# JiangongChen/ORB_SLAM3-1

Hardware: AMD Instinct MI355X
Metric: tracking frames/s (ORB extract+match) (higher is better)
Workload: dtype u8; 1 GPU; ORBextractor 640x480, 8 levels, 1000 features (configs[1]) + SearchByBoW 1000x1000 per frame (configs[2]); batch_per_gpu=256

## Files before the change

### include/orbslam3_hip.h

```cpp
#ifndef ORBSLAM3_HIP_H
#define ORBSLAM3_HIP_H

#include <stddef.h>
#include <stdint.h>

#ifdef __cplusplus
extern "C" {
#endif

#define ORBX_OK 0
#define ORBX_ERR_EMPTY (-1)
#define ORBX_ERR_CAPACITY (-2)
#define ORBX_ERR_ARG (-3)
#define ORBX_ERR_NO_DEVICE (-4)
#define ORBX_ERR_HIP (-5)
#define ORBX_ERR_INTERNAL (-6)

const char* orbx_last_error(void);
int orbx_device_count(void);


typedef struct OrbxKeyPoint {
    float x, y;
    float size;
// ... 19 lines not shown
                              int row_stride, size_t frame_stride, int lap0, int lap1,
                              OrbxKeyPoint* d_kps, uint8_t* d_desc, int cap, int32_t* d_n, int32_t* d_mono,
                              int32_t* d_status, void* stream);

int orbx_max_keypoints(const orbx_extractor* h);
int orbx_max_keypoints_for(const orbx_extractor* h, int width, int height);

int orbx_levels(const orbx_extractor* h);
float orbx_scale_factor(const orbx_extractor* h);
int orbx_scale_tables(const orbx_extractor* h, float* scale, float* inv_scale, float* sigma2, float* inv_sigma2);
int orbx_features_per_level(const orbx_extractor* h, int* n_per_level);

int orbx_pyramid_level_size(const orbx_extractor* h, int level, int* width, int* height);
int orbx_pyramid_level(orbx_extractor* h, int frame, int level, int border, uint8_t* dst, int dst_stride);

int orbx_stereo_matches(orbx_extractor* left, orbx_extractor* right, int frame,
                        const OrbxKeyPoint* kps_l, const uint8_t* desc_l, int n_l,
                        const OrbxKeyPoint* kps_r, const uint8_t* desc_r, int n_r, float mb, float mbf, float* u_right, float* depth);
int orbx_stereo_matches_device(orbx_extractor* left, orbx_extractor* right, int batch,
                               const OrbxKeyPoint* d_kps_l, const uint8_t* d_desc_l, const int32_t* d_n_l,
                               const OrbxKeyPoint* d_kps_r, const uint8_t* d_desc_r, const int32_t* d_n_r, int cap,
                               float mb, float mbf, float* d_u_right, float* d_depth, void* stream);

int orbx_profile_enable(orbx_extractor* h, int on);
int orbx_profile_read(orbx_extractor* h, float* stage_ms, int n_stages);

int orbx_debug_blurred_level(orbx_extractor* h, int frame, int level, uint8_t* dst, int dst_stride);
int orbx_debug_candidates(orbx_extractor* h, int frame, int level, OrbxKeyPoint* out, int cap, int* n);
int orbx_debug_level_keypoints(orbx_extractor* h, int frame, int level, OrbxKeyPoint* out, int cap, int* n);
int orbx_debug_set_fast_corner_cap(orbx_extractor* h, int cap);
int orbx_debug_set_tail_delay(orbx_extractor* h, int microseconds);
int orbx_debug_last_schedule(orbx_extractor* h);
int orbx_debug_fast_scores(const uint8_t* patches, int n, int pitch, int* out);


int orbm_hamming(const uint8_t a[32], const uint8_t b[32]);

typedef struct OrbmFeatVec {
    int32_t n_nodes;
    const uint32_t* node_id;
    const int32_t* offset;
    const uint32_t* feat;
} OrbmFeatVec;

typedef struct orbm_matcher orbm_matcher;
int orbm_create(int device, orbm_matcher** out);
void orbm_destroy(orbm_matcher* m);

int orbm_search_by_bow(orbm_matcher* m,
                       const uint8_t* desc_kf, int n_kf, const uint8_t* valid_kf, const float* angle_kf, const OrbmFeatVec* fv_kf,
                       const uint8_t* desc_f, int n_f, const float* angle_f, const OrbmFeatVec* fv_f,
                       float nnratio, int check_orientation, int32_t* match_f2kf);

typedef struct OrbmBowPair {
    const uint8_t* desc_kf; int32_t n_kf; const uint8_t* valid_kf; const float* angle_kf; OrbmFeatVec fv_kf;
    const uint8_t* desc_f;  int32_t n_f;  const float* angle_f;  OrbmFeatVec fv_f;
    int32_t* match_f2kf;
    int32_t n_matches;
} OrbmBowPair;
int orbm_search_by_bow_batch(orbm_matcher* m, OrbmBowPair* pairs, int n_pairs, float nnratio, int check_orientation);

typedef struct orbm_bow_plan orbm_bow_plan;
int orbm_bow_plan_create(orbm_matcher* m, const OrbmBowPair* pairs, int n_pairs, orbm_bow_plan** out);
int orbm_bow_plan_run(orbm_bow_plan* plan, float nnratio, int check_orientation, void* stream);
int orbm_bow_plan_fetch(orbm_bow_plan* plan, OrbmBowPair* pairs, void* stream);
void orbm_bow_plan_destroy(orbm_bow_plan* plan);
// ... 485 lines not shown
```

### orb_slam3-1_amd/capi.py

```python
import ctypes as C
import os

import numpy as np

_PKG_DIR = os.path.dirname(os.path.abspath(__file__))
_LIB_PATH = os.path.join(_PKG_DIR, "liborbslam3_hip.so")

KP_DTYPE = np.dtype([("x", "f4"), ("y", "f4"), ("size", "f4"), ("angle", "f4"), ("response", "f4"),
                     ("octave", "i4"), ("class_id", "i4")])
assert KP_DTYPE.itemsize == 28

ORBX_OK, ORBX_ERR_EMPTY, ORBX_ERR_CAPACITY, ORBX_ERR_ARG, ORBX_ERR_NO_DEVICE, ORBX_ERR_HIP, ORBX_ERR_INTERNAL = 0, -1, -2, -3, -4, -5, -6


class OrbxError(RuntimeError):
    def __init__(self, code, msg):
        super().__init__("orbslam3_hip error %d: %s" % (code, msg))
        self.code = code


class FeatVec(C.Structure):
    _fields_ = [("n_nodes", C.c_int32), ("node_id", C.c_void_p), ("offset", C.c_void_p), ("feat", C.c_void_p)]


# ... 29 lines not shown
    if not os.path.exists(_LIB_PATH):
        raise ImportError("%s not found: build it with __graft_entry__.build() (hipcc, gfx950). "
                          "There is no CPU fallback." % _LIB_PATH)
    return C.CDLL(_LIB_PATH)


lib = _load()
lib.orbx_last_error.restype = C.c_char_p
lib.orbx_create.argtypes = [C.c_int, C.c_float, C.c_int, C.c_int, C.c_int, C.c_int, C.POINTER(C.c_void_p)]
lib.orbx_destroy.argtypes = [C.c_void_p]
lib.orbx_extract.argtypes = [C.c_void_p, C.c_void_p, C.c_int, C.c_int, C.c_int, C.c_int, C.c_int,
                             C.c_void_p, C.c_void_p, C.c_int, C.POINTER(C.c_int), C.POINTER(C.c_int)]
lib.orbx_extract_batch.argtypes = [C.c_void_p, C.POINTER(C.c_void_p), C.c_int, C.c_int, C.c_int, C.c_int, C.c_int, C.c_int,
                                   C.c_void_p, C.c_void_p, C.c_int, C.c_void_p, C.c_void_p]
lib.orbx_extract_batch_device.argtypes = [C.c_void_p, C.c_void_p, C.c_int, C.c_int, C.c_int, C.c_int, C.c_size_t, C.c_int, C.c_int,
                                          C.c_void_p, C.c_void_p, C.c_int, C.c_void_p, C.c_void_p, C.c_void_p, C.c_void_p]
lib.orbx_max_keypoints.argtypes = [C.c_void_p]
lib.orbx_max_keypoints_for.argtypes = [C.c_void_p, C.c_int, C.c_int]
lib.orbx_levels.argtypes = [C.c_void_p]
lib.orbx_scale_factor.argtypes = [C.c_void_p]
lib.orbx_scale_factor.restype = C.c_float
lib.orbx_scale_tables.argtypes = [C.c_void_p] + [C.c_void_p] * 4
lib.orbx_features_per_level.argtypes = [C.c_void_p, C.c_void_p]
lib.orbx_pyramid_level_size.argtypes = [C.c_void_p, C.c_int, C.POINTER(C.c_int), C.POINTER(C.c_int)]
lib.orbx_pyramid_level.argtypes = [C.c_void_p, C.c_int, C.c_int, C.c_int, C.c_void_p, C.c_int]
lib.orbx_debug_blurred_level.argtypes = [C.c_void_p, C.c_int, C.c_int, C.c_void_p, C.c_int]
lib.orbx_debug_candidates.argtypes = [C.c_void_p, C.c_int, C.c_int, C.c_void_p, C.c_int, C.POINTER(C.c_int)]
lib.orbx_debug_level_keypoints.argtypes = [C.c_void_p, C.c_int, C.c_int, C.c_void_p, C.c_int, C.POINTER(C.c_int)]
lib.orbx_debug_set_tail_delay.argtypes = [C.c_void_p, C.c_int]
lib.orbx_debug_last_schedule.argtypes = [C.c_void_p]
lib.orbx_debug_introsort.argtypes = [C.c_void_p, C.c_void_p, C.c_void_p, C.c_int]
lib.orbx_debug_wave_sort.argtypes = [C.c_void_p, C.c_void_p, C.c_void_p, C.c_int]
lib.orbx_debug_fast_scores.argtypes = [C.c_void_p, C.c_int, C.c_int, C.c_void_p]
lib.orbx_debug_fast_atan2.restype = C.c_float
lib.orbx_debug_fast_atan2.argtypes = [C.c_float, C.c_float]
lib.orbx_debug_sincos.argtypes = [C.c_float, C.POINTER(C.c_float), C.POINTER(C.c_float)]


def _p(a):
    return None if a is None else a.ctypes.data_as(C.c_void_p)


def _check(code):
    if code < 0:
        raise OrbxError(code, (lib.orbx_last_error() or b"").decode())
    return code


def device_count():
    return lib.orbx_device_count()


class Extractor:

    def __init__(self, nfeatures=1000, scale_factor=1.2, nlevels=8, ini_th_fast=20, min_th_fast=7, device=0):
        h = C.c_void_p()
        _check(lib.orbx_create(nfeatures, scale_factor, nlevels, ini_th_fast, min_th_fast, device, C.byref(h)))
        self._h = h
        self.nlevels = nlevels
        self.max_keypoints = lib.orbx_max_keypoints(h)

    def close(self):
        if getattr(self, "_h", None):
            lib.orbx_destroy(self._h)
            self._h = None

# ... 1895 lines not shown
```

### orb_slam3-1_amd/csrc/orbx_device.h

```cpp
#pragma once

#include <stddef.h>
#include <stdint.h>

#include "../../include/orbslam3_hip.h"

namespace orbx {

constexpr int kEdge = 19;
constexpr int kHalfPatch = 15;
constexpr int kPatch = 31;
constexpr int kMaxLevels = 16;
constexpr int kOctLogFactor = 6;

struct LevelDesc {
    int32_t w, h, stride;
    int32_t nfeat;
    int64_t off;
    int32_t cell_begin, cell_count;
    int32_t cand_off, cand_cap;
    int32_t sel_off, sel_cap;
    float scale;
    int32_t patch_size;
};

struct CellDesc {
    int16_t level;
    int16_t x0, y0, x1, y1;
    int32_t slot_off, slot_cap;
};

struct TileDesc {
    int16_t level, x0, y0;
    int16_t edge;
};

struct __attribute__((aligned(16))) ResizeRow {
    uint32_t sy, b0, b1, pad;
};

__host__ __device__ inline int xcd_grid(int n_items) { return 8 * ((n_items + 7) / 8); }
__host__ __device__ inline int xcd_remap(int block, int grid, int frame)
{
    const int chunk = grid >> 3;
    return (((block & 7) + frame) & 7) * chunk + (block >> 3);
}

__host__ __device__ inline uint32_t pack_key(uint32_t x, uint32_t y, uint32_t resp) { return (x << 20) | (y << 8) | resp; }
__host__ __device__ inline uint32_t key_x(uint32_t e) { return e >> 20; }
__host__ __device__ inline uint32_t key_y(uint32_t e) { return (e >> 8) & 0xFFFu; }
__host__ __device__ inline uint32_t key_resp(uint32_t e) { return e & 0xFFu; }

}
```

### orb_slam3-1_amd/csrc/orbx_extractor.hip

```cpp
#include <hip/hip_runtime.h>

#include <algorithm>
#include <cmath>
#include <cstdarg>
#include <cstdio>
#include <cstdlib>
#include <cstring>
#include <string>
#include <vector>

#include "hip_check.h"
#include "orbx_kernels.hip"

namespace orbx {

thread_local std::string g_last_error;

int fail(int code, const char* fmt, ...)
{
    char buf[512];
    va_list ap;
    va_start(ap, fmt);
    vsnprintf(buf, sizeof(buf), fmt, ap);
    va_end(ap);
// ... 32 lines not shown
    {
        if (count <= n) return ORBX_OK;
        if (p) { (void)hipFree(p); p = nullptr; n = 0; }
        ORBX_HIP(hipMalloc((void**)&p, count * sizeof(T)));
        n = count;
        return ORBX_OK;
    }
    int upload(const std::vector<T>& v)
    {
        int r = ensure(v.size() ? v.size() : 1);
        if (r) return r;
        if (!v.empty()) ORBX_HIP(hipMemcpy(p, v.data(), v.size() * sizeof(T), hipMemcpyHostToDevice));
        return ORBX_OK;
    }
    void release() { if (p) (void)hipFree(p); p = nullptr; n = 0; }
};

}

using namespace orbx;

struct orbx_extractor {
    int device = 0;
    int nfeatures = 0, nlevels = 0, ini_th = 0, min_th = 0;
    float scale_factor_f = 0;
    double scale_factor_d = 0;
    std::vector<float> scale, inv_scale, sigma2, inv_sigma2;
    std::vector<int> nfeat;
    int taps[7];
    int max_kp = 0;

    int geo_w = 0, geo_h = 0;
    std::vector<LevelDesc> levels;
    std::vector<CellDesc> cells;
    std::vector<TileDesc> tiles;
    size_t pyr_frame_bytes = 0;
    int cand_frame_entries = 0, sel_frame_entries = 0;
    std::vector<StripDesc> strips;
    std::vector<StripRec> strip_recs;
    FastLds fast_layout;
    int fast_corner_cap = 0;
    size_t fast_lds = 0, oct_lds = 0;
    int oct_pool = 0, oct_lds_keys = 0, oct_small_keys = 0;
    bool oct_nodes_hbm = false;
    size_t oct_node_stride = 0;
    size_t oct_small_lds = 0;
    int oct_dyn_keys = 0;
    size_t oct_dyn_lds = 0;
    bool oct_keys_forced = false;

    DevBuf<LevelDesc> d_levels;
    DevBuf<CellDesc> d_cells;
    DevBuf<TileDesc> d_tiles;
    DevBuf<StripRec> d_strips;
    std::vector<DevBuf<int> > d_qsx0;
    std::vector<DevBuf<uint4> > d_qsel, d_qalpha;
    std::vector<DevBuf<ResizeRow> > d_rows;
    std::vector<DevBuf<int> > d_xofs, d_yofs;
    std::vector<DevBuf<short> > d_ialpha, d_ibeta;
    std::vector<uint8_t> resize_generic;

    int batch_cap = 0, last_batch = 0;
    DevBuf<uint8_t> d_pyr, d_blur;
    DevBuf<uint32_t> d_cand, d_scratch, d_sel;
    DevBuf<uint8_t> d_oct_nodes;
    DevBuf<int> d_cell_count, d_sel_count, d_kp_dst;
// ... 186 lines not shown
                qsx0[q] = xofs[4 * q];
                uint32_t se[4], al[4];
                for (int k = 0; k < 4; k++) {
                    const int dx = 4 * q + k;
                    if (dx < L.w) {
                        const int o = xofs[dx] - qsx0[q];
                        if (o < 0) return fail(ORBX_ERR_INTERNAL, "resize table: source offset %d", o);
                        if (o > 6) { resize_generic[l] = 1; se[k] = 0x0C0C0C0Cu; al[k] = 0u; continue; }
                        se[k] = (uint32_t)o | 0x0C000C00u | ((uint32_t)(o + 1) << 16);
                        al[k] = (uint32_t)(uint16_t)ia[2 * dx] | ((uint32_t)(uint16_t)ia[2 * dx + 1] << 16);
                    } else { se[k] = 0x0C0C0C0Cu; al[k] = 0u; }
                }
                qsel[q] = make_uint4(se[0], se[1], se[2], se[3]);
                qal[q] = make_uint4(al[0], al[1], al[2], al[3]);
            }
            std::vector<ResizeRow> rows((size_t)round_up(L.h, kResizeRows));
            for (size_t dy = 0; dy < rows.size(); dy++) {
                const int y = std::min((int)dy, L.h - 1);
                const int sy0 = std::min(std::max(yofs[y], 0), P.h - 1), sy1 = std::min(std::max(yofs[y] + 1, 0), P.h - 1);
                if (ib[2 * y] < 0 || ib[2 * y] > 2048 || ib[2 * y + 1] < 0 || ib[2 * y + 1] > 2048)
                    return fail(ORBX_ERR_INTERNAL, "resize table: row coefficients %d %d", ib[2 * y], ib[2 * y + 1]);
                rows[dy].sy = (uint32_t)sy0 | ((uint32_t)sy1 << 16);
                rows[dy].b0 = (uint32_t)ib[2 * y] << 12; rows[dy].b1 = (uint32_t)ib[2 * y + 1] << 12; rows[dy].pad = 0;
            }
            int r;
            if (resize_generic[l] && ((r = d_xofs[l].upload(xofs)) || (r = d_ialpha[l].upload(ia)) || (r = d_yofs[l].upload(yofs)) || (r = d_ibeta[l].upload(ib)))) return r;
            if ((r = d_qsx0[l].upload(qsx0)) || (r = d_qsel[l].upload(qsel)) || (r = d_qalpha[l].upload(qal)) || (r = d_rows[l].upload(rows))) return r;
        }
    }
    pyr_frame_bytes = off;
    if (off >= ((size_t)1 << 31)) return fail(ORBX_ERR_ARG, "the pyramid of a %dx%d image exceeds 2 GiB per frame", w, h);
    cand_frame_entries = std::max(cand_off, 1);
    sel_frame_entries = sel_off;
    {
        if (cells.size() > 32767) return fail(ORBX_ERR_ARG, "%zu FAST cells exceed the strip table's 16-bit cell index", cells.size());
        int max_nch = 1, max_ngx = 1, max_sth = 7, max_ent = 1, max_ncell = 1, max_int = 1;
        for (const StripDesc& sd : strips) {
            const int g0 = (sd.x0 + 3) >> 2, g1 = (sd.x1 - 4) >> 2, ngx = g1 - g0 + 1, sth = sd.y1 - sd.y0, ih = sth - 6;
            if (ngx > 64 || ih > 127) return fail(ORBX_ERR_ARG, "FAST strip of %dx%d px exceeds the 64-quad x 127-row work item index", sd.x1 - sd.x0, sth);
            const int xa = (4 * (g0 - 1)) & ~15, qoff = 4 * g0 - xa;
            max_nch = std::max(max_nch, (qoff + 4 * ngx + 4 + 15) >> 4);
            for (int j = 0; j < sd.ncell; j++) { const CellDesc& c = cells[sd.cell0 + j]; max_int = std::max(max_int, (c.x1 - c.x0 - 6) * ih); }
            max_ngx = std::max(max_ngx, ngx); max_sth = std::max(max_sth, sth);
            max_ent = std::max(max_ent, ((ih + 3) / 4) * (ngx + sd.ncell - 1));
            max_ncell = std::max(max_ncell, (int)sd.ncell);
        }
        if (max_int > 8191) return fail(ORBX_ERR_ARG, "FAST cell interior of %d px exceeds the 8191-px bitmask", max_int);
        FastLds& Z = fast_layout;
        auto al16 = [](size_t v) { return (v + 15) & ~(size_t)15; };
        size_t o = 0;
        Z.tile_pitch = 16 * max_nch;
        o = al16((size_t)max_sth * Z.tile_pitch);
        Z.map_off = (int)o; Z.map_pitch = 4 * max_ngx + 8;
        o = al16(o + (size_t)(max_sth - 6 + 2) * Z.map_pitch);
        Z.ent_cap = (max_ent + 7) & ~7;
        Z.ent_off = (int)o; o = al16(o + 2 * 4 * (size_t)Z.ent_cap);
        Z.px_off = (int)o; o = al16(o + 2 * 4 * (size_t)kPxCap);
        Z.corner_cap = fast_corner_cap > 0 ? fast_corner_cap : kCornerCap;
        Z.corner_off = (int)o; o = al16(o + 2 * 4 * (size_t)Z.corner_cap);
        Z.wpc = (max_int + 31) / 32;
        Z.pre_off = (int)o; o = al16(o + 4 * (size_t)max_ncell * Z.wpc);
        Z.bits_off = (int)o; o = al16(o + 4 * (size_t)max_ncell * Z.wpc);
        Z.total = (int)o;
        fast_lds = o;
        if (fast_lds > 150 * 1024) return fail(ORBX_ERR_ARG, "FAST strip of %d quads x %d rows does not fit LDS", max_ngx, max_sth);
        strip_recs.assign(strips.size(), StripRec());
// ... 237 lines not shown
            if (n_cells > 0) launch_fast(s, 0, (int)strips.size());
        }
        ORBX_LAUNCHED("k_fast_strips");
        if (marks) mark();
        hipStream_t os = blur_s ? blur_s : s;
        if (blur_s) {
            ORBX_HIP(hipEventRecord(ev_fork, s));
            ORBX_HIP(hipStreamWaitEvent(blur_s, ev_fork, 0));
        }
        if (two_launches) {
            ORBX_HIP(hipStreamWaitEvent(oct_stream, ev_fork, 0));
            {
                const int k_hi = dyn_keys ? std::max(64, o_keys / 2) : 0;
                launch_octree(oct_stream, oct_split, nlevels, oct_lds_hi + 8 * (size_t)k_hi, oct_pool_hi, k_hi);
            }
            ORBX_HIP(hipEventRecord(ev_oct_join, oct_stream));
        }
        launch_octree(os, oct0_early ? 1 : 0, lv_lo, o_lds, oct_pool, o_keys);
        if (blur_s) {
            if (tail_beside) ORBX_HIP(hipStreamWaitEvent(s, ev_tail, 0));
            launch_blur(s);
        }
        last_octree_variant = (oct_nodes_hbm ? 0 : (dyn_keys ? 3 : (o_keys > 0 ? 1 : 2))) | (two_launches ? 4 : 0) | (oct0_early ? 8 : 0) | (in_place ? 16 : 0) | (tail_beside ? 32 : 0) | (chain_beside ? 64 : 0);
        if (two_launches) ORBX_HIP(hipStreamWaitEvent(os, ev_oct_join, 0));
        ORBX_LAUNCHED("k_octree / k_blur");
        if (marks) mark();
        hipLaunchKernelGGL(k_index, dim3(nB), dim3(64), 0, os, d_levels.p, nlevels, sel, sel_frame_entries, sel_cnt,
                           lap0, lap1, cap, kp_dst, sel_frame_entries, o_n + f0, o_mono + f0, o_status + f0);
        ORBX_LAUNCHED("k_index");
        if (marks) mark();
        if (blur_s) { ORBX_HIP(hipEventRecord(ev_join, blur_s)); ORBX_HIP(hipStreamWaitEvent(s, ev_join, 0)); }
        else launch_blur(s);
        if (marks) mark();
        hipLaunchKernelGGL(k_orient_desc, dim3((unsigned)(((long long)quads * nB + 7) / 8 * 8)), dim3(256), 0, s, pyr, blr, pyr_frame_bytes,
                           d_levels.p, nlevels, sel, sel_frame_entries, sel_cnt, kp_dst, sel_frame_entries,
                           o_kps + (size_t)f0 * cap, o_desc + (size_t)f0 * cap * 32, cap, d_lvl_kps.p + (size_t)f0 * sel_frame_entries, quads, nB);
        ORBX_LAUNCHED("k_orient_desc");
        if (marks) mark();
        return ORBX_OK;
    };

    int parts = 1;
    if (!profile && split_parts > 1 && B >= 32 * split_parts) parts = std::min(split_parts, 1 + (int)aux_streams.size());
    int r;
    if (parts == 1) {
        if ((r = run_range(0, B, st, (!profile && !serial_schedule && side_stream && B >= 32) ? side_stream : nullptr, true))) return r;
    } else {
        ORBX_HIP(hipEventRecord(ev_parts_fork, st));
        for (int p = 0; p < parts; p++) {
            const int f0 = (int)((long long)B * p / parts), f1 = (int)((long long)B * (p + 1) / parts);
            hipStream_t s = p == 0 ? st : aux_streams[p - 1];
            if (p > 0) ORBX_HIP(hipStreamWaitEvent(s, ev_parts_fork, 0));
            if ((r = run_range(f0, f1 - f0, s, nullptr, false))) return r;
            if (p > 0) { ORBX_HIP(hipEventRecord(ev_parts_join[p - 1], s)); ORBX_HIP(hipStreamWaitEvent(st, ev_parts_join[p - 1], 0)); }
        }
    }
    prof_marks = mark_i;
    prof_stream = st;
    ORBX_HIP(hipGetLastError());
    last_batch = B;
    return ORBX_OK;
}

extern "C" {

int orbx_profile_enable(orbx_extractor* e, int on)
{
    if (!e) return fail(ORBX_ERR_ARG, "NULL handle");
    ORBX_HIP(hipSetDevice(e->device));
// ... 333 lines not shown
    }
    if (!r && hipMemcpy(v.data(), d, sizeof(SortNode) * n, hipMemcpyDeviceToHost) != hipSuccess) r = ORBX_ERR_HIP;
    (void)hipFree(d);
    if (r) return fail(r, "device sort failed");
    for (int i = 0; i < n; i++) { count[i] = v[i].count; ulx[i] = v[i].ulx; node[i] = v[i].node; }
    return ORBX_OK;
}

int orbx_debug_fast_scores(const uint8_t* patches, int n, int pitch, int* out)
{
    if (n < 0 || n > (1 << 22)) return fail(ORBX_ERR_ARG, "n %d outside 0..2^22", n);
    if (pitch < 8 || pitch > 1024) return fail(ORBX_ERR_ARG, "pitch %d outside 8..1024", pitch);
    if (n == 0) return ORBX_OK;
    if (!patches || !out) return fail(ORBX_ERR_ARG, "NULL argument");
    const int per_band = std::min(pitch / 8, 64), bands = (64 + per_band - 1) / per_band;
    const size_t lds = (size_t)bands * 7 * pitch;
    uint8_t* d_in = nullptr;
    int* d_out = nullptr;
    ORBX_HIP(hipMalloc(&d_in, (size_t)n * 49));
    int r = ORBX_OK;
    if (hipMalloc(&d_out, sizeof(int) * (size_t)n) != hipSuccess) r = ORBX_ERR_HIP;
    if (!r && hipMemcpy(d_in, patches, (size_t)n * 49, hipMemcpyHostToDevice) != hipSuccess) r = ORBX_ERR_HIP;
    if (!r) {
        hipLaunchKernelGGL(k_debug_fast_scores, dim3((n + 63) / 64), dim3(64), lds, 0, d_in, n, pitch, per_band, d_out);
        if (hipGetLastError() != hipSuccess || hipDeviceSynchronize() != hipSuccess) r = ORBX_ERR_HIP;
    }
    if (!r && hipMemcpy(out, d_out, sizeof(int) * (size_t)n, hipMemcpyDeviceToHost) != hipSuccess) r = ORBX_ERR_HIP;
    (void)hipFree(d_in);
    (void)hipFree(d_out);
    if (r) return fail(r, "device score tree failed");
    return ORBX_OK;
}

static int stereo_enqueue(orbx_extractor* l, orbx_extractor* r, int frame0, int batch,
                          const OrbxKeyPoint* d_kps_l, const uint8_t* d_desc_l, const int32_t* d_n_l,
                          const OrbxKeyPoint* d_kps_r, const uint8_t* d_desc_r, const int32_t* d_n_r, int cap,
                          float mb, float mbf, float* d_u_right, float* d_depth, hipStream_t st)
{
    if (l->geo_w == 0 || l->geo_w != r->geo_w || l->geo_h != r->geo_h || l->nlevels != r->nlevels || l->scale_factor_f != r->scale_factor_f)
        return fail(ORBX_ERR_ARG, "the two extractors do not hold pyramids of the same geometry");
    if (l->device != r->device) return fail(ORBX_ERR_ARG, "the two extractors live on different devices");
    if (frame0 < 0 || batch < 1 || frame0 + batch > l->last_batch || frame0 + batch > r->last_batch) return fail(ORBX_ERR_ARG, "frames outside the last extract call");
    if (l->nlevels > 16) return fail(ORBX_ERR_ARG, "more than 16 pyramid levels");
    if (cap < 1 || cap > 8192) return fail(ORBX_ERR_ARG, "cap %d outside 1..8192", cap);
    if (!(mb > 0.f) || !(mbf > 0.f)) return fail(ORBX_ERR_ARG, "mb and mbf must be positive");
    int rr = l->d_sad.ensure((size_t)batch * cap);
    if (rr) return rr;
    StereoTables T;
    for (int i = 0; i < 16; i++) { T.scale[i] = l->scale[std::min(i, l->nlevels - 1)]; T.inv_scale[i] = l->inv_scale[std::min(i, l->nlevels - 1)]; }
    const uint8_t* pl = l->d_pyr.p + (size_t)frame0 * l->pyr_frame_bytes;
    const uint8_t* pr = r->d_pyr.p + (size_t)frame0 * r->pyr_frame_bytes;
    hipLaunchKernelGGL(k_stereo_match, dim3((cap + 3) / 4, batch), dim3(256), 0, st, pl, pr, l->pyr_frame_bytes, l->d_levels.p, T,
                       d_kps_l, d_desc_l, d_n_l, d_kps_r, d_desc_r, d_n_r, cap, mb, mbf, l->nlevels, d_u_right, d_depth, l->d_sad.p);
    int n_pow2 = 2;
    while (n_pow2 < cap) n_pow2 <<= 1;
    hipLaunchKernelGGL(k_stereo_median, dim3(batch), dim3(256), (size_t)n_pow2 * sizeof(int), st, d_n_l, cap, n_pow2, d_u_right, d_depth, l->d_sad.p);
    ORBX_HIP(hipGetLastError());
    return ORBX_OK;
}

int orbx_stereo_matches_device(orbx_extractor* left, orbx_extractor* right, int batch,
                               const OrbxKeyPoint* d_kps_l, const uint8_t* d_desc_l, const int32_t* d_n_l,
                               const OrbxKeyPoint* d_kps_r, const uint8_t* d_desc_r, const int32_t* d_n_r, int cap,
                               float mb, float mbf, float* d_u_right, float* d_depth, void* stream)
{
    if (!left || !right || !d_kps_l || !d_desc_l || !d_n_l || !d_kps_r || !d_desc_r || !d_n_r || !d_u_right || !d_depth) return fail(ORBX_ERR_ARG, "NULL argument");
// ... 61 lines not shown
```

### orb_slam3-1_amd/csrc/orbx_kernels.hip

```cpp
#include <hip/hip_runtime.h>
#include <stdint.h>

#include "orbx_device.h"
#include "orbx_introsort.h"
#include "orbx_math.h"

namespace orbx {

__device__ __align__(16) const signed char d_pattern[1024] = {
#include "orb_pattern_31.inc"
};

typedef unsigned short us2 __attribute__((ext_vector_type(2)));
__device__ __forceinline__ us2 as_us2(uint32_t v) { return __builtin_bit_cast(us2, v); }
__device__ __forceinline__ uint32_t as_u32(us2 v) { return __builtin_bit_cast(uint32_t, v); }

struct SrcImage {
    const uint8_t* base;
    size_t frame_stride;
    int32_t stride, w, h;
};

__device__ __forceinline__ uint32_t mul_hi_u24(uint32_t a, uint32_t b) { return (uint32_t)(((uint64_t)(a & 0xFFFFFFu) * (uint64_t)(b & 0xFFFFFFu)) >> 32); }

// ... 700 lines not shown
        if (q_in && 2 * pm + 32 < rows_in + 6) blur_h_item(sp + 32 * SP, hp + 16 * kBlurTW, tapA, tapB);
    }
    __syncthreads();
    {
        BlurTaps c;
        c.e0 = as_us2((uint32_t)t0 | ((uint32_t)t1 << 16)); c.e1 = as_us2((uint32_t)t2 | ((uint32_t)t3 << 16));
        c.e2 = as_us2((uint32_t)t2 | ((uint32_t)t1 << 16)); c.e3 = as_us2((uint32_t)t0);
        c.o0 = as_us2((uint32_t)t0 << 16); c.o1 = as_us2((uint32_t)t1 | ((uint32_t)t2 << 16));
        c.o2 = as_us2((uint32_t)t3 | ((uint32_t)t2 << 16)); c.o3 = as_us2((uint32_t)t1 | ((uint32_t)t0 << 16));
        const uint32_t* hp = s_hp + pm * kBlurTW + 4 * q;
        const uint32_t off = __umul24((uint32_t)(y0 + 2 * pm), ostride) + (uint32_t)(x0 + 4 * q);
        if (q_in && 2 * pm < rows_in) blur_v_item(hp, c, dst, off, ostride, 2 * pm + 1 < rows_in);
        if (q_in && 2 * pm + 32 < rows_in) blur_v_item(hp + 16 * kBlurTW, c, dst, off + 32u * ostride, ostride, 2 * pm + 33 < rows_in);
    }
}

struct IcMask { uint32_t m[32][8]; };
constexpr IcMask make_ic_mask()
{
    IcMask t{};
    const int um[16] = {15, 15, 15, 15, 14, 14, 14, 13, 13, 12, 11, 10, 9, 8, 6, 3};
    for (int r = 0; r < 31; r++) {
        const int v = r - 15, av = v < 0 ? -v : v;
        for (int j = 0; j < 8; j++)
            for (int k = 0; k < 4; k++) {
                const int u = -15 + 4 * j + k, au = u < 0 ? -u : u;
                if (u <= 15 && au <= um[av]) t.m[r][j] |= 0xFFu << (8 * k);
            }
    }
    return t;
}
__device__ const IcMask d_ic_mask = make_ic_mask();

__global__ __launch_bounds__(256) void k_orient_desc(const uint8_t* __restrict__ pyr, const uint8_t* __restrict__ blur, size_t frame_stride,
                                                     const LevelDesc* __restrict__ levels, int n_levels,
                                                     const uint32_t* __restrict__ sel, int sel_frame_stride,
                                                     const int* __restrict__ sel_count,
                                                     const int* __restrict__ kp_dst, int kp_frame_stride,
                                                     OrbxKeyPoint* __restrict__ kps, uint8_t* __restrict__ desc, int cap,
                                                     OrbxKeyPoint* __restrict__ lvl_kps ,
                                                     int quads_per_frame, int batch)
{
    constexpr int kBR = 18, kBP = 64, kPR = 15;
    constexpr int kBBytes = (2 * kBR + 1) * kBP;
    __shared__ __align__(16) uint8_t s_patch[8][kBBytes];
    const int total_wg = gridDim.x, per_xcd = total_wg >> 3;
    const int v_id = (int)(blockIdx.x & 7) * per_xcd + (int)(blockIdx.x >> 3);
    const int frame = v_id / quads_per_frame, quad = v_id - frame * quads_per_frame;
    if (frame >= batch) return;
    const int lane = threadIdx.x & 63, wave = __builtin_amdgcn_readfirstlane(threadIdx.x >> 6);
    const int half = lane >> 5, hl = lane & 31;
    const int s_pair = quad * 8 + wave * 2, s_flat = s_pair + half;
    int level = 0;
    for (int l = 1; l < n_levels; l++) level = (s_pair >= levels[l].sel_off) ? l : level;
    const LevelDesc L = levels[level];
    const int k = s_flat - L.sel_off;
    const bool live = s_flat < sel_frame_stride && k < L.sel_cap && k < sel_count[(size_t)frame * n_levels + level];
    const int slot = L.sel_off + (live ? k : 0);
    const uint32_t e = live ? sel[(size_t)frame * sel_frame_stride + slot] : 0u;
    const int row = live ? kp_dst[(size_t)frame * kp_frame_stride + slot] : -1;
    uint32_t pw[8];
#pragma unroll
    for (int q = 0; q < 8; q++) pw[q] = ((const uint32_t*)d_pattern)[hl + 32 * q];
    const int px = (int)key_x(e) + 16, py = (int)key_y(e) + 16;
    uint8_t* sb = s_patch[wave * 2 + half];
    const int xb = (px - kBR) & ~15;
    uint32_t icw[9];
#pragma unroll
    for (int j = 0; j < 9; j++) icw[j] = 0u;
    if (live) {
        const uint8_t* bbase = blur + (size_t)frame * frame_stride + L.off + (size_t)(py - kBR) * L.stride + xb;
        for (int i = hl; i < (2 * kBR + 1) * 4; i += 32) {
            const int r = i >> 2, c = i & 3;
            *(uint4*)(sb + r * kBP + 16 * c) = *(const uint4*)(bbase + (size_t)r * L.stride + 16 * c);
        }
        if (hl < 2 * kPR + 1) {
            const uint8_t* rp = pyr + (size_t)frame * frame_stride + L.off + (size_t)(py - kPR + hl) * L.stride + ((px - kPR) & ~3);
            const Dwords4 q0 = *(const Dwords4*)rp, q1 = *(const Dwords4*)(rp + 16);
            icw[0] = q0.x; icw[1] = q0.y; icw[2] = q0.z; icw[3] = q0.w; icw[4] = q1.x; icw[5] = q1.y; icw[6] = q1.z; icw[7] = q1.w;
            icw[8] = *(const uint32_t*)(rp + 32);
        }
    }
    __builtin_amdgcn_fence(__ATOMIC_RELEASE, "wavefront");
    __builtin_amdgcn_wave_barrier();
    __builtin_amdgcn_fence(__ATOMIC_ACQUIRE, "wavefront");
    if (__ballot(live) == 0ull) return;

    int m10 = 0, m01 = 0;
    if (live && hl < 2 * kPR + 1) {
        const uint32_t sh = (uint32_t)((px - kPR) & 3);
        const uint4 ma = *(const uint4*)&d_ic_mask.m[hl][0], mb = *(const uint4*)&d_ic_mask.m[hl][4];
        const uint32_t mk[8] = {ma.x, ma.y, ma.z, ma.w, mb.x, mb.y, mb.z, mb.w};
        uint32_t a = 0u, b = 0u;
#pragma unroll
        for (int j = 0; j < 8; j++) {
            const uint32_t d = __builtin_amdgcn_alignbyte(icw[j + 1], icw[j], sh) & mk[j];
            a = __builtin_amdgcn_udot4(d, 0x01010101u, a, false);
            b = __builtin_amdgcn_udot4(d, 0x03020100u + 0x04040404u * (uint32_t)j, b, false);
        }
        m10 = (int)b - 15 * (int)a;
        m01 = (hl - kPR) * (int)a;
    }
    for (int o = 16; o > 0; o >>= 1) { m10 += __shfl_xor(m10, o); m01 += __shfl_xor(m01, o); }
    const float angle = fast_atan2_deg((float)m01, (float)m10);

    const float factorPI = (float)(3.141592653589793238462643383279502884 / 180.f);
    float a, b;
    sincos_f32(angle * factorPI, &a, &b);
    const uint8_t* bimg = sb + kBR * kBP + (px - xb);
    unsigned long long w[8];
#pragma unroll
    for (int q = 0; q < 8; q++) {
        const float x0 = (float)(signed char)(pw[q] & 0xFF), y0 = (float)(signed char)((pw[q] >> 8) & 0xFF);
        const float x1 = (float)(signed char)((pw[q] >> 16) & 0xFF), y1 = (float)(signed char)(pw[q] >> 24);
        int t0 = 0, t1 = 0;
        if (live) {
            t0 = bimg[cv_round_f(x0 * b + y0 * a) * kBP + cv_round_f(x0 * a - y0 * b)];
            t1 = bimg[cv_round_f(x1 * b + y1 * a) * kBP + cv_round_f(x1 * a - y1 * b)];
        }
        w[q] = __ballot(t0 < t1);
    }
    if (!live) return;
    if (hl == 0) {
        OrbxKeyPoint kp;
        kp.x = (float)px; kp.y = (float)py;
        kp.size = (float)L.patch_size; kp.angle = angle; kp.response = (float)key_resp(e);
        kp.octave = level; kp.class_id = -1;
        if (lvl_kps) lvl_kps[(size_t)frame * sel_frame_stride + slot] = kp;
        if (level != 0) { kp.x = kp.x * L.scale; kp.y = kp.y * L.scale; }
        if (row >= 0 && row < cap) kps[(size_t)frame * cap + row] = kp;
    }
    if (hl < 8 && row >= 0 && row < cap) {
        unsigned long long mine = w[0];
#pragma unroll
        for (int q = 1; q < 8; q++) mine = (hl == q) ? w[q] : mine;
        ((uint32_t*)(desc + ((size_t)frame * cap + row) * 32))[hl] = (uint32_t)(mine >> (32 * half));
    }
}

struct StereoTables { float scale[16], inv_scale[16]; };

__global__ __launch_bounds__(256) void k_stereo_match(const uint8_t* __restrict__ pyrL, const uint8_t* __restrict__ pyrR, size_t frame_stride,
                                                     const LevelDesc* __restrict__ levels, StereoTables T,
                                                     const OrbxKeyPoint* __restrict__ kpsL, const uint8_t* __restrict__ descL, const int32_t* __restrict__ nL,
                                                     const OrbxKeyPoint* __restrict__ kpsR, const uint8_t* __restrict__ descR, const int32_t* __restrict__ nR,
                                                     int cap, float mb, float mbf, int n_levels,
                                                     float* __restrict__ u_right, float* __restrict__ depth, int32_t* __restrict__ sad_out)
{
    __shared__ uint8_t s_l[4][11 * 12], s_r[4][11 * 24];
    __shared__ int s_part[4][11 * 11];
    const int frame = blockIdx.y, lane = threadIdx.x & 63, wave = threadIdx.x >> 6;
    const int iL = blockIdx.x * 4 + wave;
// ... 151 lines not shown
```

Baseline: 287,300 frames/s.

## Restructure orient/descriptor kernel: constant level table, magic divide, packed steering math

Passes per-level parameters as a by-value kernel argument table instead of a global LevelDesc array, and replaces the frame division with a magic-number multiply-high. Patch loads are restructured into five independent 16-byte loads per lane issued before a single wait, with unconditional sel/kp_dst reads clamped in range. The steering computation uses packed FP32 multiply/add with a magic-constant rounding trick so the sample address is formed from the float bit pattern, replacing cv_round and per-point multiplies. The goal is fewer scalar loads, less latency serialization and fewer VALU ops, at the cost of inline asm and a rounding mode that could differ from cv_round on ties. A debug entry point for validating the steering is also added.

After: 289,500 frames/s (median of 6 runs). About the same (+0.8%).

```diff
diff --git a/include/orbslam3_hip.h b/include/orbslam3_hip.h
--- a/include/orbslam3_hip.h
+++ b/include/orbslam3_hip.h
@@ -75,6 +75,7 @@
 int orbx_debug_set_tail_delay(orbx_extractor* h, int microseconds);
 int orbx_debug_last_schedule(orbx_extractor* h);
 int orbx_debug_fast_scores(const uint8_t* patches, int n, int pitch, int* out);
+int orbx_debug_steer(const float* ab, int n, int* out);
 
 
 int orbm_hamming(const uint8_t a[32], const uint8_t b[32]);
diff --git a/orb_slam3-1_amd/capi.py b/orb_slam3-1_amd/capi.py
--- a/orb_slam3-1_amd/capi.py
+++ b/orb_slam3-1_amd/capi.py
@@ -85,6 +85,7 @@
 lib.orbx_debug_introsort.argtypes = [C.c_void_p, C.c_void_p, C.c_void_p, C.c_int]
 lib.orbx_debug_wave_sort.argtypes = [C.c_void_p, C.c_void_p, C.c_void_p, C.c_int]
 lib.orbx_debug_fast_scores.argtypes = [C.c_void_p, C.c_int, C.c_int, C.c_void_p]
+lib.orbx_debug_steer.argtypes = [C.c_void_p, C.c_int, C.c_void_p]
 lib.orbx_debug_fast_atan2.restype = C.c_float
 lib.orbx_debug_fast_atan2.argtypes = [C.c_float, C.c_float]
 lib.orbx_debug_sincos.argtypes = [C.c_float, C.POINTER(C.c_float), C.POINTER(C.c_float)]
diff --git a/orb_slam3-1_amd/csrc/orbx_device.h b/orb_slam3-1_amd/csrc/orbx_device.h
--- a/orb_slam3-1_amd/csrc/orbx_device.h
+++ b/orb_slam3-1_amd/csrc/orbx_device.h
@@ -39,6 +39,19 @@
     uint32_t sy, b0, b1, pad;
 };
 
+struct __attribute__((aligned(32))) OrientLevel {
+    int32_t sel_off, sel_cap;
+    uint32_t off;
+    int32_t stride;
+    float scale;
+    int32_t patch_size;
+    int32_t pad[2];
+};
+struct OrientTab {
+    int32_t sel_off[kMaxLevels];
+    OrientLevel lv[kMaxLevels];
+};
+
 __host__ __device__ inline int xcd_grid(int n_items) { return 8 * ((n_items + 7) / 8); }
 __host__ __device__ inline int xcd_remap(int block, int grid, int frame)
 {
diff --git a/orb_slam3-1_amd/csrc/orbx_extractor.hip b/orb_slam3-1_amd/csrc/orbx_extractor.hip
--- a/orb_slam3-1_amd/csrc/orbx_extractor.hip
+++ b/orb_slam3-1_amd/csrc/orbx_extractor.hip
@@ -88,6 +88,7 @@
 
     int geo_w = 0, geo_h = 0;
     std::vector<LevelDesc> levels;
+    OrientTab orient_tab;
     std::vector<CellDesc> cells;
     std::vector<TileDesc> tiles;
     size_t pyr_frame_bytes = 0;
@@ -340,6 +341,15 @@
     if (off >= ((size_t)1 << 31)) return fail(ORBX_ERR_ARG, "the pyramid of a %dx%d image exceeds 2 GiB per frame", w, h);
     cand_frame_entries = std::max(cand_off, 1);
     sel_frame_entries = sel_off;
+    std::memset(&orient_tab, 0, sizeof(orient_tab));
+    for (int l = 0; l < kMaxLevels; l++) {
+        orient_tab.sel_off[l] = INT32_MAX;
+        if (l >= nlevels) continue;
+        const LevelDesc& L = levels[l];
+        OrientLevel& O = orient_tab.lv[l];
+        orient_tab.sel_off[l] = L.sel_off;
+        O.sel_off = L.sel_off; O.sel_cap = L.sel_cap; O.off = (uint32_t)L.off; O.stride = L.stride; O.scale = L.scale; O.patch_size = L.patch_size;
+    }
     {
         if (cells.size() > 32767) return fail(ORBX_ERR_ARG, "%zu FAST cells exceed the strip table's 16-bit cell index", cells.size());
         int max_nch = 1, max_ngx = 1, max_sth = 7, max_ent = 1, max_ncell = 1, max_int = 1;
@@ -643,9 +653,13 @@
         if (blur_s) { ORBX_HIP(hipEventRecord(ev_join, blur_s)); ORBX_HIP(hipStreamWaitEvent(s, ev_join, 0)); }
         else launch_blur(s);
         if (marks) mark();
-        hipLaunchKernelGGL(k_orient_desc, dim3((unsigned)(((long long)quads * nB + 7) / 8 * 8)), dim3(256), 0, s, pyr, blr, pyr_frame_bytes,
-                           d_levels.p, nlevels, sel, sel_frame_entries, sel_cnt, kp_dst, sel_frame_entries,
-                           o_kps + (size_t)f0 * cap, o_desc + (size_t)f0 * cap * 32, cap, d_lvl_kps.p + (size_t)f0 * sel_frame_entries, quads, nB);
+        {
+            const unsigned od_grid = (unsigned)(((long long)quads * nB + 7) / 8 * 8);
+            const uint32_t quad_magic = (quads > 1 && (uint64_t)od_grid * (uint64_t)quads < (1ull << 32)) ? (uint32_t)(((1ull << 32) + quads - 1) / quads) : 0u;
+            hipLaunchKernelGGL(k_orient_desc, dim3(od_grid), dim3(256), 0, s, pyr, blr, pyr_frame_bytes,
+                               orient_tab, nlevels, sel, sel_frame_entries, sel_cnt, kp_dst, sel_frame_entries,
+                               o_kps + (size_t)f0 * cap, o_desc + (size_t)f0 * cap * 32, cap, d_lvl_kps.p + (size_t)f0 * sel_frame_entries, quads, quad_magic, nB);
+        }
         ORBX_LAUNCHED("k_orient_desc");
         if (marks) mark();
         return ORBX_OK;
@@ -1045,6 +1059,28 @@
     return ORBX_OK;
 }
 
+int orbx_debug_steer(const float* ab, int n, int* out)
+{
+    if (n < 0 || n > (1 << 20)) return fail(ORBX_ERR_ARG, "n %d outside 0..2^20", n);
+    if (n == 0) return ORBX_OK;
+    if (!ab || !out) return fail(ORBX_ERR_ARG, "NULL argument");
+    float2* d_in = nullptr;
+    int* d_out = nullptr;
+    ORBX_HIP(hipMalloc(&d_in, sizeof(float2) * (size_t)n));
+    int r = ORBX_OK;
+    if (hipMalloc(&d_out, sizeof(int) * 1024 * (size_t)n) != hipSuccess) r = ORBX_ERR_HIP;
+    if (!r && hipMemcpy(d_in, ab, sizeof(float2) * (size_t)n, hipMemcpyHostToDevice) != hipSuccess) r = ORBX_ERR_HIP;
+    if (!r) {
+        hipLaunchKernelGGL(k_debug_steer, dim3(n), dim3(256), 0, 0, d_in, d_out);
+        if (hipGetLastError() != hipSuccess || hipDeviceSynchronize() != hipSuccess) r = ORBX_ERR_HIP;
+    }
+    if (!r && hipMemcpy(out, d_out, sizeof(int) * 1024 * (size_t)n, hipMemcpyDeviceToHost) != hipSuccess) r = ORBX_ERR_HIP;
+    (void)hipFree(d_in);
+    (void)hipFree(d_out);
+    if (r) return fail(r, "device steering failed");
+    return ORBX_OK;
+}
+
 static int stereo_enqueue(orbx_extractor* l, orbx_extractor* r, int frame0, int batch,
                           const OrbxKeyPoint* d_kps_l, const uint8_t* d_desc_l, const int32_t* d_n_l,
                           const OrbxKeyPoint* d_kps_r, const uint8_t* d_desc_r, const int32_t* d_n_r, int cap,
diff --git a/orb_slam3-1_amd/csrc/orbx_kernels.hip b/orb_slam3-1_amd/csrc/orbx_kernels.hip
--- a/orb_slam3-1_amd/csrc/orbx_kernels.hip
+++ b/orb_slam3-1_amd/csrc/orbx_kernels.hip
@@ -756,54 +756,111 @@
 }
 __device__ const IcMask d_ic_mask = make_ic_mask();
 
+typedef float f32x2 __attribute__((ext_vector_type(2)));
+constexpr uint32_t kRoundBits = 0x4B400000u;
+__device__ __forceinline__ uint2 steer_bits(f32x2 xy, f32x2 ba, f32x2 magic)
+{
+    f32x2 p, q, s, r;
+    asm("v_pk_mul_f32 %0, %1, %2 op_sel_hi:[0,1]" : "=v"(p) : "v"(xy), "v"(ba));
+    asm("v_pk_mul_f32 %0, %1, %2 op_sel:[1,1] op_sel_hi:[1,0]" : "=v"(q) : "v"(xy), "v"(ba));
+    asm("v_pk_add_f32 %0, %1, %2 neg_hi:[0,1]" : "=v"(s) : "v"(p), "v"(q));
+    asm("v_pk_add_f32 %0, %1, %2" : "=v"(r) : "v"(s), "v"(magic));
+    return make_uint2(__float_as_uint(r.x), __float_as_uint(r.y));
+}
+
+__global__ __launch_bounds__(256) void k_debug_steer(const float2* __restrict__ ab, int* __restrict__ out)
+{
+    const float2 v = ab[blockIdx.x];
+    const f32x2 ba = {v.y, v.x}, magic = {12582912.f, 12582912.f};
+    const uint32_t pw = ((const uint32_t*)d_pattern)[threadIdx.x];
+    const f32x2 xy0 = {(float)(signed char)(pw & 0xFF), (float)(signed char)((pw >> 8) & 0xFF)};
+    const f32x2 xy1 = {(float)(signed char)((pw >> 16) & 0xFF), (float)(signed char)(pw >> 24)};
+    const uint2 r0 = steer_bits(xy0, ba, magic), r1 = steer_bits(xy1, ba, magic);
+    int4 o;
+    o.x = (int)(r0.x - kRoundBits); o.y = (int)(r0.y - kRoundBits); o.z = (int)(r1.x - kRoundBits); o.w = (int)(r1.y - kRoundBits);
+    ((int4*)out)[(size_t)blockIdx.x * 256 + threadIdx.x] = o;
+}
+
 __global__ __launch_bounds__(256) void k_orient_desc(const uint8_t* __restrict__ pyr, const uint8_t* __restrict__ blur, size_t frame_stride,
-                                                     const LevelDesc* __restrict__ levels, int n_levels,
+                                                     OrientTab T, int n_levels,
                                                      const uint32_t* __restrict__ sel, int sel_frame_stride,
                                                      const int* __restrict__ sel_count,
                                                      const int* __restrict__ kp_dst, int kp_frame_stride,
                                                      OrbxKeyPoint* __restrict__ kps, uint8_t* __restrict__ desc, int cap,
                                                      OrbxKeyPoint* __restrict__ lvl_kps ,
-                                                     int quads_per_frame, int batch)
+                                                     int quads_per_frame, uint32_t quad_magic, int batch)
 {
     constexpr int kBR = 18, kBP = 64, kPR = 15;
     constexpr int kBBytes = (2 * kBR + 1) * kBP;
-    __shared__ __align__(16) uint8_t s_patch[8][kBBytes];
-    const int total_wg = gridDim.x, per_xcd = total_wg >> 3;
-    const int v_id = (int)(blockIdx.x & 7) * per_xcd + (int)(blockIdx.x >> 3);
-    const int frame = v_id / quads_per_frame, quad = v_id - frame * quads_per_frame;
+    __shared__ __align__(16) uint8_t s_patch[8 * kBBytes];
+    const uint32_t total_wg = gridDim.x;
+    {
+        typedef int i32x4 __attribute__((ext_vector_type(4)));
+        const i32x4* so = (const i32x4*)T.sel_off;
+        asm volatile("" : : "s"(pyr), "s"(blur), "s"(frame_stride), "s"(so[0]), "s"(so[1]), "s"(so[2]), "s"(so[3]), "s"(n_levels), "s"(sel),
+                     "s"(sel_frame_stride), "s"(sel_count), "s"(kp_dst), "s"(kp_frame_stride), "s"(kps), "s"(desc), "s"(cap), "s"(lvl_kps),
+                     "s"(quads_per_frame), "s"(quad_magic), "s"(batch), "s"(total_wg));
+    }
+    const uint32_t per_xcd = total_wg >> 3;
+    const uint32_t v_id = (blockIdx.x & 7u) * per_xcd + (blockIdx.x >> 3);
+    const int frame = (int)(quad_magic ? __umulhi(v_id, quad_magic) : v_id / (uint32_t)quads_per_frame);
+    const int quad = (int)v_id - frame * quads_per_frame;
     if (frame >= batch) return;
     const int lane = threadIdx.x & 63, wave = __builtin_amdgcn_readfirstlane(threadIdx.x >> 6);
     const int half = lane >> 5, hl = lane & 31;
+    uint32_t pw[8];
+#pragma unroll
+    for (int q = 0; q < 8; q++) pw[q] = ((const uint32_t*)d_pattern)[hl + 32 * q];
+    const uint4 ma = *(const uint4*)&d_ic_mask.m[hl][0], mb = *(const uint4*)&d_ic_mask.m[hl][4];
     const int s_pair = quad * 8 + wave * 2, s_flat = s_pair + half;
-    int level = 0;
-    for (int l = 1; l < n_levels; l++) level = (s_pair >= levels[l].sel_off) ? l : level;
-    const LevelDesc L = levels[level];
-    const int k = s_flat - L.sel_off;
-    const bool live = s_flat < sel_frame_stride && k < L.sel_cap && k < sel_count[(size_t)frame * n_levels + level];
-    const int slot = L.sel_off + (live ? k : 0);
-    const uint32_t e = live ? sel[(size_t)frame * sel_frame_stride + slot] : 0u;
-    const int row = live ? kp_dst[(size_t)frame * kp_frame_stride + slot] : -1;
-    uint32_t pw[8];
-#pragma unroll
-    for (int q = 0; q < 8; q++) pw[q] = ((const uint32_t*)d_pattern)[hl + 32 * q];
+    int level = 0, lvl_off = T.sel_off[0];
+#pragma unroll
+    for (int l = 1; l < kMaxLevels; l++) {
+        const bool ge = s_pair >= T.sel_off[l];
+        level = ge ? l : level;
+        lvl_off = ge ? T.sel_off[l] : lvl_off;
+    }
+    const bool in_range = s_flat < sel_frame_stride;
+    const int s_read = min(s_flat, sel_frame_stride - 1);
+    const uint32_t e_any = sel[(size_t)frame * sel_frame_stride + s_read];
+    const int row_any = kp_dst[(size_t)frame * kp_frame_stride + s_read];
+    const int count = sel_count[(size_t)frame * n_levels + level];
+    const OrientLevel L = T.lv[level];
+    asm volatile("" : : "s"(L.sel_cap), "s"(L.off), "s"(L.stride), "s"(L.scale), "s"(L.patch_size));
+    const int k = s_flat - lvl_off;
+    const bool live = in_range & (k < L.sel_cap) & (k < count);
+    const int slot = s_flat;
+    const uint32_t e = live ? e_any : 0u;
+    const int row = live ? row_any : -1;
     const int px = (int)key_x(e) + 16, py = (int)key_y(e) + 16;
-    uint8_t* sb = s_patch[wave * 2 + half];
+    const uint32_t sb = __umul24((uint32_t)(wave * 2 + half), (uint32_t)kBBytes);
     const int xb = (px - kBR) & ~15;
     uint32_t icw[9];
-#pragma unroll
-    for (int j = 0; j < 9; j++) icw[j] = 0u;
     if (live) {
-        const uint8_t* bbase = blur + (size_t)frame * frame_stride + L.off + (size_t)(py - kBR) * L.stride + xb;
-        for (int i = hl; i < (2 * kBR + 1) * 4; i += 32) {
-            const int r = i >> 2, c = i & 3;
-            *(uint4*)(sb + r * kBP + 16 * c) = *(const uint4*)(bbase + (size_t)r * L.stride + 16 * c);
-        }
-        if (hl < 2 * kPR + 1) {
-            const uint8_t* rp = pyr + (size_t)frame * frame_stride + L.off + (size_t)(py - kPR + hl) * L.stride + ((px - kPR) & ~3);
-            const Dwords4 q0 = *(const Dwords4*)rp, q1 = *(const Dwords4*)(rp + 16);
-            icw[0] = q0.x; icw[1] = q0.y; icw[2] = q0.z; icw[3] = q0.w; icw[4] = q1.x; icw[5] = q1.y; icw[6] = q1.z; icw[7] = q1.w;
-            icw[8] = *(const uint32_t*)(rp + 32);
-        }
+        const uint32_t stride = (uint32_t)L.stride;
+        const uint8_t* bb = blur + (size_t)frame * frame_stride + L.off;
+        const uint8_t* pb = pyr + (size_t)frame * frame_stride + L.off;
+        const uint32_t bo = __umul24((uint32_t)(py - kBR + (hl >> 2)), stride) + (uint32_t)(xb + 16 * (hl & 3));
+        const uint32_t po = __umul24((uint32_t)(py - kPR + hl), stride) + (uint32_t)((px - kPR) & ~3);
+        const bool fifth = hl < (2 * kBR + 1) * 4 - 128, ic_row = hl < 2 * kPR + 1;
+        uint4 c0, c1, c2, c3, c4;
+        Dwords4 q0, q1;
+        uint32_t q2 = 0u;
+        c0 = *(const uint4*)(bb + bo);
+        c1 = *(const uint4*)(bb + (size_t)(8u * stride) + bo);
+        c2 = *(const uint4*)(bb + (size_t)(16u * stride) + bo);
+        c3 = *(const uint4*)(bb + (size_t)(24u * stride) + bo);
+        if (fifth) c4 = *(const uint4*)(bb + (size_t)(32u * stride) + bo);
+        if (ic_row) {
+            q0 = *(const Dwords4*)(pb + po); q1 = *(const Dwords4*)(pb + 16 + po);
+            q2 = *(const uint32_t*)(pb + 32 + po);
+        }
+        __builtin_amdgcn_s_waitcnt(0x0F70);
+        uint8_t* sw = s_patch + sb + 16 * hl;
+        *(uint4*)sw = c0; *(uint4*)(sw + 512) = c1; *(uint4*)(sw + 1024) = c2; *(uint4*)(sw + 1536) = c3;
+        if (fifth) *(uint4*)(sw + 2048) = c4;
+        icw[0] = q0.x; icw[1] = q0.y; icw[2] = q0.z; icw[3] = q0.w; icw[4] = q1.x; icw[5] = q1.y; icw[6] = q1.z; icw[7] = q1.w;
+        icw[8] = q2;
     }
     __builtin_amdgcn_fence(__ATOMIC_RELEASE, "wavefront");
     __builtin_amdgcn_wave_barrier();
@@ -813,7 +870,6 @@
     int m10 = 0, m01 = 0;
     if (live && hl < 2 * kPR + 1) {
         const uint32_t sh = (uint32_t)((px - kPR) & 3);
-        const uint4 ma = *(const uint4*)&d_ic_mask.m[hl][0], mb = *(const uint4*)&d_ic_mask.m[hl][4];
         const uint32_t mk[8] = {ma.x, ma.y, ma.z, ma.w, mb.x, mb.y, mb.z, mb.w};
         uint32_t a = 0u, b = 0u;
 #pragma unroll
@@ -831,17 +887,16 @@
     const float factorPI = (float)(3.141592653589793238462643383279502884 / 180.f);
     float a, b;
     sincos_f32(angle * factorPI, &a, &b);
-    const uint8_t* bimg = sb + kBR * kBP + (px - xb);
+    const f32x2 ba = {b, a}, magic = {12582912.f, 12582912.f};
+    const uint32_t sbase = sb + (uint32_t)(kBR * kBP + (px - xb)) - kRoundBits * (uint32_t)(kBP + 1);
     unsigned long long w[8];
 #pragma unroll
     for (int q = 0; q < 8; q++) {
-        const float x0 = (float)(signed char)(pw[q] & 0xFF), y0 = (float)(signed char)((pw[q] >> 8) & 0xFF);
-        const float x1 = (float)(signed char)((pw[q] >> 16) & 0xFF), y1 = (float)(signed char)(pw[q] >> 24);
-        int t0 = 0, t1 = 0;
-        if (live) {
-            t0 = bimg[cv_round_f(x0 * b + y0 * a) * kBP + cv_round_f(x0 * a - y0 * b)];
-            t1 = bimg[cv_round_f(x1 * b + y1 * a) * kBP + cv_round_f(x1 * a - y1 * b)];
-        }
+        const f32x2 xy0 = {(float)(signed char)(pw[q] & 0xFF), (float)(signed char)((pw[q] >> 8) & 0xFF)};
+        const f32x2 xy1 = {(float)(signed char)((pw[q] >> 16) & 0xFF), (float)(signed char)(pw[q] >> 24)};
+        const uint2 r0 = steer_bits(xy0, ba, magic), r1 = steer_bits(xy1, ba, magic);
+        const int t0 = s_patch[(r0.x << 6) + r0.y + sbase];
+        const int t1 = s_patch[(r1.x << 6) + r1.y + sbase];
         w[q] = __ballot(t0 < t1);
     }
     if (!live) return;
```
